# snuspl/parallax

Hardware: NVIDIA H100
Metric: lm1b_words_per_sec (higher is better)
Workload: dtype bf16

## Files before the change

parallax_b200/ops/csrc/kernels/lstm_softmax.cu:

```cuda
#include "common.cuh"

template <typename T> __device__ __forceinline__ float to_f(T v);
template <> __device__ __forceinline__ float to_f<float>(float v) { return v; }
template <> __device__ __forceinline__ float to_f<__nv_bfloat16>(__nv_bfloat16 v) { return __bfloat162float(v); }
template <typename T> __device__ __forceinline__ T from_f(float v);
template <> __device__ __forceinline__ float from_f<float>(float v) { return v; }
template <> __device__ __forceinline__ __nv_bfloat16 from_f<__nv_bfloat16>(float v) { return __float2bfloat16_rn(v); }

__device__ __forceinline__ float sigmoidf_(float x) { return 1.f / (1.f + __expf(-x)); }
__device__ __forceinline__ float tanhf_(float x) {
  const float e = __expf(-2.f * fabsf(x));
  const float t = (1.f - e) / (1.f + e);
  return copysignf(t, x);
}

template <typename T>
__global__ void __launch_bounds__(256)
px_lstm_cell_fwd_kernel(const T* __restrict__ gates, const float* __restrict__ c_prev,
                        T* __restrict__ act, float* __restrict__ c_new, T* __restrict__ m,
                        int B, int S, float forget_bias) {
  const int total = B * S;
  for (int idx = blockIdx.x * blockDim.x + threadIdx.x; idx < total;
       idx += gridDim.x * blockDim.x) {
    const int b = idx / S, s = idx - b * S;
    const size_t g0 = (size_t)b * 4 * S + s;
    const float si = sigmoidf_(to_f(gates[g0]));
    const float tj = tanhf_(to_f(gates[g0 + S]));
    const float sf = sigmoidf_(to_f(gates[g0 + 2 * S]) + forget_bias);
    const float so = sigmoidf_(to_f(gates[g0 + 3 * S]));
    const float c = sf * c_prev[idx] + si * tj;
    c_new[idx] = c;
    m[idx] = from_f<T>(so * tanhf_(c));
    act[g0] = from_f<T>(si);
    act[g0 + S] = from_f<T>(tj);
    act[g0 + 2 * S] = from_f<T>(sf);
    act[g0 + 3 * S] = from_f<T>(so);
  }
}

template <typename T>
__global__ void __launch_bounds__(256)
px_lstm_cell_bwd_kernel(const T* __restrict__ dm, float* __restrict__ dc,
                        const T* __restrict__ act, const float* __restrict__ c_prev,
                        const float* __restrict__ c_new, T* __restrict__ dgates, int B, int S) {
  const int total = B * S;
  for (int idx = blockIdx.x * blockDim.x + threadIdx.x; idx < total;
       idx += gridDim.x * blockDim.x) {
    const int b = idx / S, s = idx - b * S;
    const size_t g0 = (size_t)b * 4 * S + s;
    const float si = to_f(act[g0]), tj = to_f(act[g0 + S]), sf = to_f(act[g0 + 2 * S]),
                so = to_f(act[g0 + 3 * S]);
    const float tc = tanhf_(c_new[idx]);
    const float dmv = to_f(dm[idx]);
    const float dcv = dc[idx] + dmv * so * (1.f - tc * tc);
    dgates[g0] = from_f<T>(dcv * tj * si * (1.f - si));
    dgates[g0 + S] = from_f<T>(dcv * si * (1.f - tj * tj));
    dgates[g0 + 2 * S] = from_f<T>(dcv * c_prev[idx] * sf * (1.f - sf));
    dgates[g0 + 3 * S] = from_f<T>(dmv * tc * so * (1.f - so));
    dc[idx] = dcv * sf;
  }
}

template <typename T, int ITEMS, bool DOT>
__global__ void __launch_bounds__(256)
px_sampled_softmax_kernel(T* __restrict__ logits, const float* __restrict__ true_dot,
                          const float* __restrict__ adj_true,
                          const float* __restrict__ adj_samp,
                          const long long* __restrict__ targets, const long long* __restrict__ sampled,
                          float* __restrict__ loss, float* __restrict__ dtrue, int N, int S,
                          const T* __restrict__ h, const T* __restrict__ w_true, int P) {
  const int row = blockIdx.x;
  if (row >= N) return;
  __shared__ float s_red[8];
  __shared__ float s_bcast;
  T* x = logits + (size_t)row * S;
  const long long tgt = targets[row];
  float tl;
  if (DOT) {
    __shared__ float s_dot[8];
    const T* hr = h + (size_t)row * P;
    const T* wr = w_true + (size_t)row * P;
    float part = 0.f;
    for (int k = threadIdx.x; k < P; k += 256) part += to_f(hr[k]) * to_f(wr[k]);
    part = warp_sum(part);
    if ((threadIdx.x & 31) == 0) s_dot[threadIdx.x >> 5] = part;
    __syncthreads();
    float t = 0.f;
#pragma unroll
    for (int k = 0; k < 8; ++k) t += s_dot[k];
    tl = t + adj_true[row];
  } else {
    tl = true_dot[row] + adj_true[row];
  }
  float v[ITEMS];
  float mx = tl;
#pragma unroll
  for (int k = 0; k < ITEMS; ++k) {
    const int j = k * 256 + threadIdx.x;
    float a = -INFINITY;
    if (j < S) {
      a = to_f(x[j]) + adj_samp[j];
      if (sampled[j] == tgt) a = -INFINITY;
    }
    v[k] = a;
    mx = fmaxf(mx, a);
  }
  for (int o = 16; o > 0; o >>= 1) mx = fmaxf(mx, __shfl_xor_sync(0xffffffffu, mx, o));
  if ((threadIdx.x & 31) == 0) s_red[threadIdx.x >> 5] = mx;
  __syncthreads();
  if (threadIdx.x < 32) {
    float t = threadIdx.x < 8 ? s_red[threadIdx.x] : -INFINITY;
    for (int o = 4; o > 0; o >>= 1) t = fmaxf(t, __shfl_xor_sync(0xffffffffu, t, o));
    if (threadIdx.x == 0) s_bcast = t;
  }
  __syncthreads();
  mx = s_bcast;
  float sum = 0.f;
#pragma unroll
  for (int k = 0; k < ITEMS; ++k) { v[k] = __expf(v[k] - mx); sum += v[k]; }
  sum = warp_sum(sum);
  __syncthreads();
  if ((threadIdx.x & 31) == 0) s_red[threadIdx.x >> 5] = sum;
  __syncthreads();
  if (threadIdx.x < 32) {
    float t = threadIdx.x < 8 ? s_red[threadIdx.x] : 0.f;
    t = warp_sum(t);
    if (threadIdx.x == 0) s_bcast = t + __expf(tl - mx);
  }
  __syncthreads();
  const float denom = s_bcast;
  const float inv = 1.f / denom;
#pragma unroll
  for (int k = 0; k < ITEMS; ++k) {
    const int j = k * 256 + threadIdx.x;
    if (j < S) x[j] = from_f<T>(v[k] * inv);
  }
  if (threadIdx.x == 0) {
    loss[row] = (mx + __logf(denom)) - tl;
    dtrue[row] = __expf(tl - mx) * inv - 1.f;
  }
}

template <typename T> struct PxVec16;
template <> struct PxVec16<float> {
  static constexpr int N = 4;
  float v[4];
  __device__ __forceinline__ void load(const float* p) {
    const float4 t = *reinterpret_cast<const float4*>(p);
    v[0] = t.x; v[1] = t.y; v[2] = t.z; v[3] = t.w;
  }
  __device__ __forceinline__ void store(float* p) const {
    *reinterpret_cast<float4*>(p) = make_float4(v[0], v[1], v[2], v[3]);
  }
};
template <> struct PxVec16<__nv_bfloat16> {
  static constexpr int N = 8;
  float v[8];
  __device__ __forceinline__ void load(const __nv_bfloat16* p) {
    const uint4 t = *reinterpret_cast<const uint4*>(p);
    const unsigned w[4] = {t.x, t.y, t.z, t.w};
#pragma unroll
    for (int i = 0; i < 4; ++i) {
      v[2 * i] = __uint_as_float(w[i] << 16);
      v[2 * i + 1] = __uint_as_float(w[i] & 0xffff0000u);
    }
  }
  __device__ __forceinline__ void store(__nv_bfloat16* p) const {
    unsigned w[4];
#pragma unroll
    for (int i = 0; i < 4; ++i) {
      const __nv_bfloat162 b = __floats2bfloat162_rn(v[2 * i], v[2 * i + 1]);
      w[i] = *reinterpret_cast<const unsigned*>(&b);
    }
    *reinterpret_cast<uint4*>(p) = make_uint4(w[0], w[1], w[2], w[3]);
  }
};

template <typename T>
__global__ void __launch_bounds__(256)
px_ssm_bwd_kernel(T* __restrict__ G, const T* __restrict__ inputs, const T* __restrict__ w_true,
                  const float* __restrict__ g, int g_stride, const float* __restrict__ row_w,
                  const float* __restrict__ dtrue, float inv_n, T* __restrict__ gi,
                  T* __restrict__ d_w_true, void* __restrict__ d_b_true, int db_bf16,
                  T* __restrict__ grow_out, int N, int P) {
  constexpr int V = PxVec16<T>::N;
  const int per_row = P / V;
  const long long total = (long long)N * per_row;
  for (long long idx = (long long)blockIdx.x * blockDim.x + threadIdx.x; idx < total;
       idx += (long long)gridDim.x * blockDim.x) {
    const int row = (int)(idx / per_row);
    const int col = (int)(idx - (long long)row * per_row);
    float grow = g[(size_t)row * g_stride] * inv_n;
    if (row_w != nullptr) grow *= row_w[row];
    const float gt = grow * dtrue[row];
    const size_t off = (size_t)row * P + (size_t)col * V;
    PxVec16<T> a, x, w, o;
    a.load(G + off);
    x.load(inputs + off);
    w.load(w_true + off);
#pragma unroll
    for (int i = 0; i < V; ++i) o.v[i] = a.v[i] * grow + gt * w.v[i];
    o.store(G + off);
#pragma unroll
    for (int i = 0; i < V; ++i) o.v[i] = x.v[i] * grow;
    o.store(gi + off);
#pragma unroll
    for (int i = 0; i < V; ++i) o.v[i] = x.v[i] * gt;
    o.store(d_w_true + off);
    if (col == 0) {
      if (db_bf16) reinterpret_cast<__nv_bfloat16*>(d_b_true)[row] = __float2bfloat16_rn(gt);
      else reinterpret_cast<float*>(d_b_true)[row] = gt;
      grow_out[row] = from_f<T>(grow);
    }
  }
}

extern "C" {

int px_lstm_cell_fwd(const void* gates, const float* c_prev, void* act, float* c_new, void* m,
                     int B, int S, float forget_bias, int dtype, cudaStream_t stream) {
  int blocks = (B * S + 255) / 256;
  if (blocks > PX_NUM_SMS * 8) blocks = PX_NUM_SMS * 8;
  if (dtype == 0)
    px_lstm_cell_fwd_kernel<float><<<blocks, 256, 0, stream>>>(
        (const float*)gates, c_prev, (float*)act, c_new, (float*)m, B, S, forget_bias);
  else
    px_lstm_cell_fwd_kernel<__nv_bfloat16><<<blocks, 256, 0, stream>>>(
        (const __nv_bfloat16*)gates, c_prev, (__nv_bfloat16*)act, c_new, (__nv_bfloat16*)m, B, S,
        forget_bias);
  return (int)cudaGetLastError();
}

int px_lstm_cell_bwd(const void* dm, float* dc, const void* act, const float* c_prev,
                     const float* c_new, void* dgates, int B, int S, int dtype, cudaStream_t stream) {
  int blocks = (B * S + 255) / 256;
  if (blocks > PX_NUM_SMS * 8) blocks = PX_NUM_SMS * 8;
  if (dtype == 0)
    px_lstm_cell_bwd_kernel<float><<<blocks, 256, 0, stream>>>(
        (const float*)dm, dc, (const float*)act, c_prev, c_new, (float*)dgates, B, S);
  else
    px_lstm_cell_bwd_kernel<__nv_bfloat16><<<blocks, 256, 0, stream>>>(
        (const __nv_bfloat16*)dm, dc, (const __nv_bfloat16*)act, c_prev, c_new,
        (__nv_bfloat16*)dgates, B, S);
  return (int)cudaGetLastError();
}

int px_sampled_softmax(void* logits, const float* true_dot, const float* adj_true,
                       const float* adj_samp, const long long* targets, const long long* sampled,
                       float* loss, float* dtrue, int N, int S, int dtype, cudaStream_t stream) {
  if (S > 256 * 64) return -2;
#define SS(T, I)                                                                          \
  px_sampled_softmax_kernel<T, I, false><<<N, 256, 0, stream>>>(                          \
      (T*)logits, true_dot, adj_true, adj_samp, targets, sampled, loss, dtrue, N, S,      \
      (const T*)nullptr, (const T*)nullptr, 0)
#define SSD(T)                                                      \
  if (S <= 256 * 4) SS(T, 4); else if (S <= 256 * 8) SS(T, 8);      \
  else if (S <= 256 * 16) SS(T, 16); else if (S <= 256 * 32) SS(T, 32); else SS(T, 64)
  if (dtype == 0) { SSD(float); } else { SSD(__nv_bfloat16); }
#undef SSD
#undef SS
  return (int)cudaGetLastError();
}

int px_sampled_softmax_dot(void* logits, const void* h, const void* w_true, int P,
                           const float* adj_true, const float* adj_samp,
                           const long long* targets, const long long* sampled, float* loss,
                           float* dtrue, int N, int S, int dtype, cudaStream_t stream) {
  if (S > 256 * 64) return -2;
#define SS(T, I)                                                                          \
  px_sampled_softmax_kernel<T, I, true><<<N, 256, 0, stream>>>(                           \
      (T*)logits, nullptr, adj_true, adj_samp, targets, sampled, loss, dtrue, N, S,       \
      (const T*)h, (const T*)w_true, P)
#define SSD(T)                                                      \
  if (S <= 256 * 4) SS(T, 4); else if (S <= 256 * 8) SS(T, 8);      \
  else if (S <= 256 * 16) SS(T, 16); else if (S <= 256 * 32) SS(T, 32); else SS(T, 64)
  if (dtype == 0) { SSD(float); } else { SSD(__nv_bfloat16); }
#undef SSD
#undef SS
  return (int)cudaGetLastError();
}

int px_ssm_bwd(void* G, const void* inputs, const void* w_true, const float* g, int g_stride,
               const float* row_w, const float* dtrue, float inv_n, void* gi, void* d_w_true,
               void* d_b_true, int db_bf16, void* grow_out, int N, int P, int dtype,
               cudaStream_t stream) {
  const int vec = dtype == 0 ? 4 : 8;
  if (P % vec) return -2;
  const long long total = (long long)N * (P / vec);
  int blocks = (int)((total + 255) / 256);
  if (blocks > PX_NUM_SMS * 8) blocks = PX_NUM_SMS * 8;
  if (blocks < 1) blocks = 1;
  if (dtype == 0)
    px_ssm_bwd_kernel<float><<<blocks, 256, 0, stream>>>(
        (float*)G, (const float*)inputs, (const float*)w_true, g, g_stride, row_w, dtrue, inv_n,
        (float*)gi, (float*)d_w_true, d_b_true, db_bf16, (float*)grow_out, N, P);
  else
    px_ssm_bwd_kernel<__nv_bfloat16><<<blocks, 256, 0, stream>>>(
        (__nv_bfloat16*)G, (const __nv_bfloat16*)inputs, (const __nv_bfloat16*)w_true, g,
        g_stride, row_w, dtrue, inv_n, (__nv_bfloat16*)gi, (__nv_bfloat16*)d_w_true, d_b_true,
        db_bf16, (__nv_bfloat16*)grow_out, N, P);
  return (int)cudaGetLastError();
}

}
```

parallax_b200/ops/fused.py:

```python
import ctypes

import torch

from . import lib as _lib, check as _check, register_signatures

_vp, _i, _f = ctypes.c_void_p, ctypes.c_int, ctypes.c_float
register_signatures({
    "px_lstm_cell_fwd": (_i, [_vp, _vp, _vp, _vp, _vp, _i, _i, _f, _i, _vp]),
    "px_lstm_cell_bwd": (_i, [_vp, _vp, _vp, _vp, _vp, _vp, _i, _i, _i, _vp]),
    "px_sampled_softmax": (_i, [_vp, _vp, _vp, _vp, _vp, _vp, _vp, _vp, _i, _i, _i, _vp]),
    "px_sampled_softmax_dot": (_i, [_vp, _vp, _vp, _i, _vp, _vp, _vp, _vp, _vp, _vp, _i, _i, _i,
                                    _vp]),
    "px_ssm_bwd": (_i, [_vp, _vp, _vp, _vp, _i, _vp, _vp, _f, _vp, _vp, _vp, _i, _vp, _i, _i, _i,
                        _vp]),
})
_DT = {torch.float32: 0, torch.bfloat16: 1}


def _p(t):
    return _vp(t.data_ptr())


def _stream():
    return _vp(torch.cuda.current_stream().cuda_stream)


def _count(n=1):
    from ..parallel import nvops
    nvops.launches["n"] += n


def _acc(t):
    return t if t.dtype == torch.float64 else t.float()


def lstm_layer_reference(x, Wx, Wh, bias, W_P, c0, h0, forget_bias=1.0):
    T, Bsz, E = x.shape
    S = W_P.shape[0]
    xw = torch.addmm(bias, x.reshape(T * Bsz, E), Wx).view(T, Bsz, 4 * S)
    c, h, outs = _acc(c0), h0, []
    for t in range(T):
        gates = _acc(torch.addmm(xw[t], h, Wh))
        i, j, f, o = gates.split(S, dim=1)
        c = torch.sigmoid(f + forget_bias) * c + torch.sigmoid(i) * torch.tanh(j)
        m = (torch.sigmoid(o) * torch.tanh(c)).to(x.dtype)
        h = m @ W_P
        outs.append(h)
    return torch.stack(outs), c, h


class _LSTMLayerFn(torch.autograd.Function):

    @staticmethod
    def forward(ctx, x, W, Wh, bias, W_P, c0, h0, forget_bias):
        L = _lib()
        T, Bsz, E = x.shape
        S, P = W_P.shape
        dt = x.dtype
        dev = x.device
        x = x.contiguous()
        stacked = Wh is None
        ctx.stacked = stacked
        ctx.param_refs = (W, bias, W_P)
        if stacked:
            Wx, Wh = W.detach()[:E], W.detach()[E:]
        else:
            Wx = W
        if any(ctx.needs_input_grad):
            from . import sinks
            cur = torch.cuda.current_stream(dev)
            ws = sinks.side_stream(dev)
            ws.wait_stream(cur)
            with torch.cuda.stream(ws):
                ctx.WPT = W_P.detach().t().contiguous()
                ctx.WPT_ev = torch.cuda.Event()
                ctx.WPT_ev.record(ws)
            ctx.WPT.record_stream(cur)
        xw = torch.addmm(bias, x.view(T * Bsz, E), Wx).view(T, Bsz, 4 * S)
        act = torch.empty(T, Bsz, 4 * S, dtype=dt, device=dev)
        c_all = torch.empty(T + 1, Bsz, S, dtype=torch.float32, device=dev)
        m_all = torch.empty(T, Bsz, S, dtype=dt, device=dev)
        h_all = torch.empty(T + 1, Bsz, P, dtype=dt, device=dev)
        c_all[0].copy_(c0)
        h_all[0].copy_(h0)
        st = _stream()
        for t in range(T):
            gpre = xw[t].addmm_(h_all[t], Wh)
            _check(L.px_lstm_cell_fwd(_p(gpre), _p(c_all[t]), _p(act[t]),
                                      _p(c_all[t + 1]), _p(m_all[t]), Bsz, S,
                                      float(forget_bias), _DT[dt], st), "lstm_cell_fwd")
            torch.mm(m_all[t], W_P, out=h_all[t + 1])
        _count(T)
        ctx.save_for_backward(x, Wx, Wh, W_P, act, c_all, m_all, h_all)
        ctx.dims = (T, Bsz, E, S, P)
        return h_all[1:], c_all[T].clone(), h_all[T].clone()

    @staticmethod
    def backward(ctx, dH, dcT, dhT):
        from . import sinks
        L = _lib()
        x, Wx, Wh, W_P, act, c_all, m_all, h_all = ctx.saved_tensors
        T, Bsz, E, S, P = ctx.dims
        stacked = ctx.stacked
        W_ref, bias_ref, WP_ref = ctx.param_refs
        dt, dev = x.dtype, x.device
        dH = dH.contiguous()
        dgates = torch.empty(T, Bsz, 4 * S, dtype=dt, device=dev)
        dh_tot = torch.empty(T, Bsz, P, dtype=dt, device=dev)
        dc = torch.zeros(Bsz, S, dtype=torch.float32, device=dev) if dcT is None \
            else dcT.float().clone()
        dh_rec = None if dhT is None else dhT.to(dt)
        dm = torch.empty(Bsz, S, dtype=dt, device=dev)
        cur = torch.cuda.current_stream(dev)
        cur.wait_event(ctx.WPT_ev)
        WPT = ctx.WPT
        from . import gemm as _gemm
        use_tc = (dt == torch.bfloat16 and Bsz % 128 == 0 and P % 64 == 0 and
                  (4 * S) % 1024 == 0 and Wh.is_contiguous())
        WhT = None if use_tc else Wh.t().contiguous()
        st = _stream()

        def sink_of(ref, shape):
            s_ = sinks.get(ref)
            if s_ is not None and s_.dtype == dt and tuple(s_.shape) == tuple(shape):
                return s_, True
            return torch.empty(shape, dtype=dt, device=dev), False
        if stacked:
            dW, w_sunk = sink_of(W_ref, (E + P, 4 * S))
            dWx_o, dWh_o = dW[:E], dW[E:]
        else:
            dWx_o, w_sunk = sink_of(W_ref, (E, 4 * S))
            dWh_o = torch.empty(P, 4 * S, dtype=dt, device=dev)
        dbias_o, b_sunk = sink_of(bias_ref, (4 * S,))
        dWP_o, p_sunk = sink_of(WP_ref, (S, P))
        ws = sinks.side_stream(dev)
        ws2 = sinks.side_stream(dev, 1)
        if dh_rec is None:
            dh_tot[T - 1].copy_(dH[T - 1])
        else:
            torch.add(dH[T - 1], dh_rec, out=dh_tot[T - 1])
        for t in range(T - 1, -1, -1):
            torch.mm(dh_tot[t], WPT, out=dm)
            _check(L.px_lstm_cell_bwd(_p(dm), _p(dc), _p(act[t]), _p(c_all[t]),
                                      _p(c_all[t + 1]), _p(dgates[t]), Bsz, S, _DT[dt], st),
                   "lstm_cell_bwd")
            if t > 0:
                if use_tc:
                    _gemm.gemm_tn(dgates[t], Wh, addend=dH[t - 1], splits=8, bn=64,
                                  out=dh_tot[t - 1])
                else:
                    torch.addmm(dH[t - 1], dgates[t], WhT, out=dh_tot[t - 1])
            else:
                dh_rec = _gemm.gemm_tn(dgates[0], Wh, splits=8, bn=64) if use_tc \
                    else torch.mm(dgates[0], WhT)
        _count(T)
        dg2 = dgates.view(T * Bsz, 4 * S)
        ws2.wait_stream(cur)
        with torch.cuda.stream(ws2):
            torch.sum(dg2, 0, out=dbias_o)
        ev_b = torch.cuda.Event()
        ev_b.record(ws2)
        dgates.record_stream(ws2)
        dbias_o.record_stream(ws2)
        dx = (dg2 @ Wx.t()).view(T, Bsz, E)
        ws.wait_stream(cur)
        with torch.cuda.stream(ws):
            torch.mm(h_all[:T].reshape(-1, P).t(), dg2, out=dWh_o)
            torch.mm(x.reshape(-1, E).t(), dg2, out=dWx_o)
            torch.mm(m_all.reshape(-1, S).t(), dh_tot.view(-1, P), out=dWP_o)
        ev = torch.cuda.Event()
        ev.record(ws)
        for t_ in (dgates, dh_tot, x, h_all, m_all, dWh_o, dWx_o, dbias_o, dWP_o):
            t_.record_stream(ws)
        outs, plain = [], False
        for ref, o, sunk, e_ in ((W_ref, dW if stacked else dWx_o, w_sunk, ev),
                                 (bias_ref, dbias_o, b_sunk, ev_b), (WP_ref, dWP_o, p_sunk, ev)):
            if sunk:
                sinks.deliver(ref, e_)
                outs.append(None)
            else:
                outs.append(o)
                plain = True
        if plain or not stacked:
            cur.wait_event(ev)
            cur.wait_event(ev_b)
        dW_out, dbias, dW_P = outs
        return dx, dW_out, None if stacked else dWh_o, dbias, dW_P, dc, dh_rec, None


def lstm_layer(x, Wx, Wh, bias, W_P, c0, h0, forget_bias=1.0):
    if x.is_cuda and x.dtype in _DT:
        return _LSTMLayerFn.apply(x, Wx, Wh, bias, W_P, c0, h0, forget_bias)
    return lstm_layer_reference(x, Wx, Wh, bias, W_P, c0, h0, forget_bias)


def lstm_layer_stacked(x, W, bias, W_P, c0, h0, forget_bias=1.0):
    E = x.shape[-1]
    if x.is_cuda and x.dtype in _DT:
        return _LSTMLayerFn.apply(x, W, None, bias, W_P, c0, h0, forget_bias)
    return lstm_layer_reference(x, W[:E], W[E:], bias, W_P, c0, h0, forget_bias)


def sampled_softmax_reference(inputs, true_w, samp_w, true_b, samp_b, logq_true,
                              logq_samp, targets, sampled):
    true_logits = _acc((inputs * true_w).sum(-1)) + _acc(true_b) - logq_true
    samp_logits = _acc(inputs @ samp_w.t()) + (_acc(samp_b) - logq_samp)
    hits = targets.unsqueeze(1) == sampled.unsqueeze(0)
    samp_logits = samp_logits.masked_fill(hits, float("-inf"))
    lse = torch.logsumexp(torch.cat([true_logits.unsqueeze(1), samp_logits], 1), 1)
    return lse - true_logits


class _SampledSoftmaxFn(torch.autograd.Function):
    @staticmethod
    def forward(ctx, inputs, true_w, samp_w, true_b, samp_b, logq_true, logq_samp,
                targets, sampled):
        L = _lib()
        N, S = inputs.shape[0], samp_w.shape[0]
        dt = inputs.dtype
        logits = inputs @ samp_w.t()
        true_dot = (inputs.float() * true_w.float()).sum(-1)
        adj_t = (true_b.float() - logq_true).contiguous()
        adj_s = (samp_b.float() - logq_samp).contiguous()
        loss = torch.empty(N, dtype=torch.float32, device=inputs.device)
        dtrue = torch.empty(N, dtype=torch.float32, device=inputs.device)
        tg = targets.to(torch.int64).contiguous()
        sm = sampled.to(torch.int64).contiguous()
        _check(L.px_sampled_softmax(_p(logits), _p(true_dot), _p(adj_t), _p(adj_s), _p(tg),
                                    _p(sm), _p(loss), _p(dtrue), N, S, _DT[dt], _stream()),
               "sampled_softmax")
        _count(1)
        ctx.save_for_backward(inputs, true_w, samp_w, logits, dtrue)
        return loss

    @staticmethod
    def backward(ctx, g):
        inputs, true_w, samp_w, probs, dtrue = ctx.saved_tensors
        dt = inputs.dtype
        g = g.float()
        gt = (g * dtrue).unsqueeze(1)
        d_inputs = ((probs @ samp_w).float() * g.unsqueeze(1) +
                    gt * true_w.float()).to(dt)
        gi = (inputs.float() * g.unsqueeze(1)).to(dt)
        d_samp_w = probs.t() @ gi
        d_true_w = (gt * inputs.float()).to(dt)
        d_samp_b = (probs.float().t() @ g) if probs.dtype == torch.float32 else \
            torch.mm(probs.t(), g.to(dt).unsqueeze(1), out_dtype=torch.float32).squeeze(1)
        d_true_b = gt.squeeze(1)
        return d_inputs, d_true_w, d_samp_w, d_true_b, d_samp_b, None, None, None, None


def sampled_softmax_loss(inputs, true_w, samp_w, true_b, samp_b, logq_true, logq_samp,
                         targets, sampled):
    if inputs.is_cuda and inputs.dtype in _DT and samp_w.shape[0] <= 256 * 64:
        return _SampledSoftmaxFn.apply(inputs, true_w.to(inputs.dtype),
                                       samp_w.to(inputs.dtype), true_b, samp_b,
                                       logq_true, logq_samp, targets, sampled)
    return sampled_softmax_reference(inputs, true_w, samp_w, true_b, samp_b, logq_true,
                                     logq_samp, targets, sampled)


def _head_forward(inputs, w_all, adj, targets, sampled):
    N, S = inputs.shape[0], w_all.shape[0] - inputs.shape[0]
    P = inputs.shape[1]
    logits = inputs @ w_all[N:].t()
    if inputs.is_cuda:
        loss = torch.empty(N, dtype=torch.float32, device=inputs.device)
        dtrue = torch.empty(N, dtype=torch.float32, device=inputs.device)
        _check(_lib().px_sampled_softmax_dot(
            _p(logits), _p(inputs), _p(w_all), P, _p(adj), _vp(adj.data_ptr() + 4 * N),
            _p(targets), _p(sampled), _p(loss), _p(dtrue), N, S, _DT[inputs.dtype], _stream()),
            "sampled_softmax_dot")
        _count(1)
        return logits, loss, dtrue
    tl = (inputs.float() * w_all[:N].float()).sum(-1) + adj[:N]
    a = logits.float() + adj[N:]
    a = a.masked_fill(targets.unsqueeze(1) == sampled.unsqueeze(0), float("-inf"))
    mx = torch.maximum(a.max(1).values, tl)
    e, et = torch.exp(a - mx.unsqueeze(1)), torch.exp(tl - mx)
    denom = e.sum(1) + et
    return (e / denom.unsqueeze(1)).to(inputs.dtype), mx + torch.log(denom) - tl, et / denom - 1.0


def _head_backward(G, inputs, w_all, g, row_w, dtrue, gi, d_w_all, db, grow):
    N, P = inputs.shape
    if inputs.is_cuda:
        _check(_lib().px_ssm_bwd(
            _p(G), _p(inputs), _p(w_all), _p(g), 0 if g.numel() == 1 else 1,
            _p(row_w) if row_w is not None else None, _p(dtrue), 1.0 / N, _p(gi), _p(d_w_all),
            _p(db), 1 if db.dtype == torch.bfloat16 else 0, _p(grow), N, P, _DT[inputs.dtype],
            _stream()), "ssm_bwd")
        _count(1)
        return
    gr = g.reshape(-1).float() * (1.0 / N)
    gr = gr.expand(N) if gr.numel() == 1 else gr
    if row_w is not None:
        gr = gr * row_w
    gt = gr * dtrue
    x, wt = inputs.float(), w_all[:N].float()
    G.copy_(G.float() * gr.unsqueeze(1) + gt.unsqueeze(1) * wt)
    gi.copy_(x * gr.unsqueeze(1))
    d_w_all[:N].copy_(x * gt.unsqueeze(1))
    db[:N].copy_(gt)
    grow.copy_(gr)


class _SampledSoftmaxHeadFn(torch.autograd.Function):

    @staticmethod
    def forward(ctx, inputs, w_all, b_all, adj, targets, sampled, row_w):
        probs, loss, dtrue = _head_forward(inputs, w_all, adj, targets, sampled)
        ctx.save_for_backward(inputs, w_all, probs, dtrue, row_w)
        ctx.b_meta = (tuple(b_all.shape), b_all.dtype)
        if row_w is not None:
            loss = loss * row_w
        return loss.mean()

    @staticmethod
    def backward(ctx, g):
        inputs, w_all, probs, dtrue, row_w = ctx.saved_tensors
        N, P = inputs.shape
        S = w_all.shape[0] - N
        dt, dev = inputs.dtype, inputs.device
        b_shape, b_dt = ctx.b_meta
        g = g.float().contiguous()
        G = probs @ w_all[N:]
        d_w_all = torch.empty(N + S, P, dtype=dt, device=dev)
        db = torch.empty(N + S, dtype=b_dt if b_dt in _DT else torch.float32, device=dev)
        gi = torch.empty(N, P, dtype=dt, device=dev)
        grow = torch.empty(N, dtype=dt, device=dev)
        _head_backward(G, inputs, w_all, g, row_w, dtrue, gi, d_w_all, db, grow)
        torch.mm(probs.t(), gi, out=d_w_all[N:])
        if db.dtype == dt:
            torch.mm(probs.t(), grow.view(N, 1), out=db[N:].view(S, 1))
        elif dt == torch.bfloat16 and db.dtype == torch.float32:
            db[N:].copy_(torch.mm(probs.t(), grow.view(N, 1), out_dtype=torch.float32).view(S))
        else:
            db[N:].copy_((probs.t() @ grow.view(N, 1)).view(S))
        db = db.view(b_shape)
        if db.dtype != b_dt:
            db = db.to(b_dt)
        return G, d_w_all, db, None, None, None, None


def sampled_softmax_head(inputs, w_all, b_all, logq, targets, sampled, row_w=None, adj=None):
    N, P = inputs.shape
    S = w_all.shape[0] - N
    dt = inputs.dtype
    vec = 4 if dt == torch.float32 else 8
    fused = (inputs.is_cuda and dt in _DT and w_all.dtype == dt and
             0 < S <= 256 * 64 and P % vec == 0 and b_all.numel() == N + S)
    if fused:
        inputs = inputs.contiguous()
        w_all = w_all.contiguous()
        fused = inputs.data_ptr() % 16 == 0 and w_all.data_ptr() % 16 == 0
    if not fused:
        b = b_all.reshape(-1)
        loss = sampled_softmax_loss(inputs, w_all[:N], w_all[N:], b[:N], b[N:], logq[:N],
                                    logq[N:], targets, sampled)
        if row_w is not None:
            loss = loss * row_w.to(loss.dtype)
        return loss.mean()
    if adj is None:
        adj = b_all.detach().reshape(-1).float() - logq
    adj = adj.float().contiguous()
    tg = targets.to(torch.int64).contiguous()
    sm = sampled.to(torch.int64).contiguous()
    rw = None if row_w is None else row_w.detach().float().contiguous()
    return _SampledSoftmaxHeadFn.apply(inputs, w_all, b_all, adj, tg, sm, rw)
```

Measured before the change: 1.864 million.

## Fuse LSTM backward recurrence into a persistent cooperative kernel with grid barriers

Replaces the per-timestep loop of three launches (dm GEMM, cell backward, dh GEMM) with one cooperative persistent kernel. Each block keeps slices of W_P and Wh resident in shared memory, computes the dm projection with mma.sync, applies the cell backward math, then does a split-K dh GEMM with a workspace reduction, using software grid barriers between phases. This removes per-step launch overhead and repeated weight reloads, in exchange for grid-wide barrier latency and shape restrictions; unsupported shapes fall back to the old loop. It also factors the cell math into a shared header.

Result: faster. 1.916 million (median of 6 runs) (+2.8%).

```diff
diff --git a/parallax_b200/ops/csrc/kernels/lstm_cell.cuh b/parallax_b200/ops/csrc/kernels/lstm_cell.cuh
--- /dev/null
+++ b/parallax_b200/ops/csrc/kernels/lstm_cell.cuh
@@ -0,0 +1,34 @@
+#pragma once
+#include "common.cuh"
+
+__device__ __forceinline__ float sigmoidf_(float x) { return 1.f / (1.f + __expf(-x)); }
+__device__ __forceinline__ float tanhf_(float x) {
+  const float e = __expf(-2.f * fabsf(x));
+  const float t = (1.f - e) / (1.f + e);
+  return copysignf(t, x);
+}
+
+__device__ __forceinline__ void lstm_cell_fwd_math(float gi, float gj, float gf, float go,
+                                                   float c_prev, float forget_bias, float& si,
+                                                   float& tj, float& sf, float& so, float& c,
+                                                   float& m) {
+  si = sigmoidf_(gi);
+  tj = tanhf_(gj);
+  sf = sigmoidf_(gf + forget_bias);
+  so = sigmoidf_(go);
+  c = sf * c_prev + si * tj;
+  m = so * tanhf_(c);
+}
+
+__device__ __forceinline__ void lstm_cell_bwd_math(float si, float tj, float sf, float so,
+                                                   float c_prev, float c_new, float dmv,
+                                                   float dc_next, float (&dg)[4],
+                                                   float& dc_prev) {
+  const float tc = tanhf_(c_new);
+  const float dcv = dc_next + dmv * so * (1.f - tc * tc);
+  dg[0] = dcv * tj * si * (1.f - si);
+  dg[1] = dcv * si * (1.f - tj * tj);
+  dg[2] = dcv * c_prev * sf * (1.f - sf);
+  dg[3] = dmv * tc * so * (1.f - so);
+  dc_prev = dcv * sf;
+}
diff --git a/parallax_b200/ops/csrc/kernels/lstm_persistent.cu b/parallax_b200/ops/csrc/kernels/lstm_persistent.cu
--- /dev/null
+++ b/parallax_b200/ops/csrc/kernels/lstm_persistent.cu
@@ -0,0 +1,360 @@
+#include <map>
+#include <mutex>
+#include <set>
+#include <tuple>
+
+#include "lstm_cell.cuh"
+
+namespace lp {
+
+constexpr int WARPS = 8;
+constexpr int THREADS = WARPS * 32;
+constexpr int CH = 64;
+constexpr int NST = 4;
+constexpr int STAGE_BYTES = 16 * CH * 2;
+constexpr int STAGING = WARPS * NST * STAGE_BYTES;
+constexpr int UNITS = 16;
+constexpr int KS_BWD = 16;
+constexpr size_t CTR_BYTES = 32 * 4;
+
+__device__ __forceinline__ uint32_t smem_u32(const void* p) {
+  return (uint32_t)__cvta_generic_to_shared(p);
+}
+__device__ __forceinline__ uint32_t swz(int r, int c, int row_chunks) {
+  return (uint32_t)((r * row_chunks + (c ^ (r & 7))) * 16);
+}
+__device__ __forceinline__ void cp_async16(uint32_t dst, const void* src) {
+  asm volatile("cp.async.cg.shared.global [%0], [%1], 16;" ::"r"(dst), "l"(src) : "memory");
+}
+__device__ __forceinline__ void cp_async_commit() {
+  asm volatile("cp.async.commit_group;" ::: "memory");
+}
+template <int N>
+__device__ __forceinline__ void cp_async_wait() {
+  asm volatile("cp.async.wait_group %0;" ::"n"(N) : "memory");
+}
+__device__ __forceinline__ void ldmatrix_x4(uint32_t addr, uint32_t (&r)[4]) {
+  asm volatile("ldmatrix.sync.aligned.m8n8.x4.shared.b16 {%0,%1,%2,%3}, [%4];"
+               : "=r"(r[0]), "=r"(r[1]), "=r"(r[2]), "=r"(r[3]) : "r"(addr));
+}
+__device__ __forceinline__ void mma_bf16(float (&d)[4], const uint32_t (&a)[4], uint32_t b0,
+                                         uint32_t b1) {
+  asm volatile(
+      "mma.sync.aligned.m16n8k16.row.col.f32.bf16.bf16.f32 "
+      "{%0,%1,%2,%3}, {%4,%5,%6,%7}, {%8,%9}, {%0,%1,%2,%3};"
+      : "+f"(d[0]), "+f"(d[1]), "+f"(d[2]), "+f"(d[3])
+      : "r"(a[0]), "r"(a[1]), "r"(a[2]), "r"(a[3]), "r"(b0), "r"(b1));
+}
+__device__ __forceinline__ float bf16r(float v) {
+  return __bfloat162float(__float2bfloat16_rn(v));
+}
+__device__ __forceinline__ float2 ld_bf16x2(const __nv_bfloat16* p) {
+  return __bfloat1622float2(*reinterpret_cast<const __nv_bfloat162*>(p));
+}
+__device__ __forceinline__ void st_bf16x2(__nv_bfloat16* p, float a, float b) {
+  *reinterpret_cast<__nv_bfloat162*>(p) = __floats2bfloat162_rn(a, b);
+}
+
+__device__ __forceinline__ void bar_sync(unsigned int* ctr, bool leader, unsigned int n) {
+  __syncthreads();
+  if (threadIdx.x == 0) {
+    const unsigned int add = leader ? 0x80000000u - (n - 1u) : 1u;
+    __threadfence();
+    const unsigned int old = atomicAdd(ctr, add);
+    unsigned int cur;
+    do {
+      asm volatile("ld.acquire.gpu.global.u32 %0, [%1];" : "=r"(cur) : "l"(ctr) : "memory");
+    } while (((old ^ cur) & 0x80000000u) == 0u);
+    __threadfence();
+  }
+  __syncthreads();
+}
+
+template <int NT>
+__device__ __forceinline__ void warp_gemm(float (&acc)[NT][4], const __nv_bfloat16* A, int lda,
+                                          int K, uint32_t ring, uint32_t bs, int b_chunks) {
+  const int lane = threadIdx.x & 31;
+#pragma unroll
+  for (int nt = 0; nt < NT; ++nt)
+#pragma unroll
+    for (int e = 0; e < 4; ++e) acc[nt][e] = 0.f;
+  const int nch = K / CH;
+  auto load = [&](int ch) {
+    const uint32_t st = ring + (ch % NST) * STAGE_BYTES;
+#pragma unroll
+    for (int i = lane; i < 16 * (CH / 8); i += 32) {
+      const int r = i / (CH / 8), c = i % (CH / 8);
+      cp_async16(st + swz(r, c, CH / 8), A + (size_t)r * lda + ch * CH + c * 8);
+    }
+  };
+#pragma unroll
+  for (int s = 0; s < NST - 1; ++s) {
+    if (s < nch) load(s);
+    cp_async_commit();
+  }
+  for (int ch = 0; ch < nch; ++ch) {
+    if (ch + NST - 1 < nch) load(ch + NST - 1);
+    cp_async_commit();
+    cp_async_wait<NST - 1>();
+    __syncwarp();
+    const uint32_t st = ring + (ch % NST) * STAGE_BYTES;
+#pragma unroll
+    for (int kk = 0; kk < CH / 16; ++kk) {
+      uint32_t a[4];
+      ldmatrix_x4(st + swz(lane & 15, kk * 2 + (lane >> 4), CH / 8), a);
+      const int kc = ch * (CH / 8) + kk * 2;
+      const int mi = lane >> 3;
+#pragma unroll
+      for (int nt = 0; nt < NT; nt += 2) {
+        uint32_t b[4];
+        ldmatrix_x4(bs + swz((nt + (mi >> 1)) * 8 + (lane & 7), kc + (mi & 1), b_chunks), b);
+        mma_bf16(acc[nt], a, b[0], b[1]);
+        mma_bf16(acc[nt + 1], a, b[2], b[3]);
+      }
+    }
+    __syncwarp();
+  }
+}
+
+__device__ __forceinline__ void load_rows(uint8_t* bs, const __nv_bfloat16* src, size_t ld,
+                                          int rows, int K) {
+  const int chunks = K / 8;
+  for (int i = threadIdx.x; i < rows * chunks; i += THREADS) {
+    const int r = i / chunks, c = i % chunks;
+    *reinterpret_cast<uint4*>(bs + swz(r, c, chunks)) =
+        *reinterpret_cast<const uint4*>(src + (size_t)r * ld + c * 8);
+  }
+}
+template <int KS>
+__device__ __forceinline__ void split_reduce(const float (&acc)[8][4], float* ws,
+                                             unsigned int* tile_ctr, int nb, int ks, int B,
+                                             int P, const __nv_bfloat16* addend,
+                                             __nv_bfloat16* out) {
+  const int warp = threadIdx.x >> 5, lane = threadIdx.x & 31;
+  if (warp * 16 < B) {
+#pragma unroll
+    for (int nt = 0; nt < 8; ++nt)
+#pragma unroll
+      for (int h = 0; h < 2; ++h) {
+        const int row = warp * 16 + (lane >> 2) + 8 * h;
+        const int col = nb * 64 + nt * 8 + 2 * (lane & 3);
+        *reinterpret_cast<float2*>(ws + ((size_t)ks * B + row) * P + col) =
+            make_float2(acc[nt][2 * h], acc[nt][2 * h + 1]);
+      }
+  }
+  bar_sync(tile_ctr, ks == 0, KS);
+  constexpr int ROWS = 128 / KS;
+  for (int v = threadIdx.x; v < ROWS * 16; v += THREADS) {
+    const int row = ks * ROWS + v / 16, col = nb * 64 + (v % 16) * 4;
+    if (row >= B) continue;
+    float4 s = make_float4(0.f, 0.f, 0.f, 0.f);
+#pragma unroll
+    for (int p = 0; p < KS; ++p) {
+      const float4 x = __ldcg(reinterpret_cast<const float4*>(ws + ((size_t)p * B + row) * P + col));
+      s.x += x.x; s.y += x.y; s.z += x.z; s.w += x.w;
+    }
+    const size_t off = (size_t)row * P + col;
+    if (addend) {
+      const float2 lo = ld_bf16x2(addend + off), hi = ld_bf16x2(addend + off + 2);
+      s.x += lo.x; s.y += lo.y; s.z += hi.x; s.w += hi.y;
+    }
+    st_bf16x2(out + off, s.x, s.y);
+    st_bf16x2(out + off + 2, s.z, s.w);
+  }
+}
+
+struct BwdArgs {
+  const __nv_bfloat16* dH;
+  const __nv_bfloat16* Wh;
+  const __nv_bfloat16* WP;
+  const __nv_bfloat16* act;
+  const float* c_all;
+  __nv_bfloat16* dgates;
+  __nv_bfloat16* dh_tot;
+  __nv_bfloat16* dh_rec;
+  float* dc;
+  float* ws;
+  unsigned int* ctr;
+  int T, B, S, P;
+};
+
+__global__ void __launch_bounds__(THREADS, 1) px_lstm_bwd_persistent_kernel(BwdArgs a) {
+  extern __shared__ __align__(128) uint8_t smem[];
+  const int j = blockIdx.x, G = gridDim.x;
+  const int warp = threadIdx.x >> 5, lane = threadIdx.x & 31;
+  const int B = a.B, S = a.S, P = a.P, S4 = 4 * S;
+  const int ntiles = P / 64, Kb = S4 / KS_BWD;
+  const bool proj = j < ntiles * KS_BWD;
+  const int nb = j % ntiles, ks = j / ntiles;
+  uint8_t* s_wp = smem;
+  uint8_t* s_wh = s_wp + UNITS * P * 2;
+  const uint32_t ring = smem_u32(s_wh + 64 * Kb * 2) + warp * NST * STAGE_BYTES;
+  load_rows(s_wp, a.WP + (size_t)UNITS * j * P, (size_t)P, UNITS, P);
+  if (proj) load_rows(s_wh, a.Wh + (size_t)nb * 64 * S4 + (size_t)ks * Kb, (size_t)S4, 64, Kb);
+  __syncthreads();
+
+  const bool rows_on = warp * 16 < B;
+  const int g = lane >> 2, q = lane & 3;
+  float dc[2][2][2];
+  if (rows_on) {
+#pragma unroll
+    for (int rr = 0; rr < 2; ++rr)
+#pragma unroll
+      for (int nt = 0; nt < 2; ++nt) {
+        const float2 v = *reinterpret_cast<const float2*>(
+            a.dc + (size_t)(warp * 16 + g + 8 * rr) * S + UNITS * j + 8 * nt + 2 * q);
+        dc[rr][nt][0] = v.x; dc[rr][nt][1] = v.y;
+      }
+  }
+  unsigned int* grid_ctr = a.ctr;
+  for (int t = a.T - 1; t >= 0; --t) {
+    if (rows_on) {
+      float acc[2][4];
+      warp_gemm<2>(acc, a.dh_tot + ((size_t)t * B + warp * 16) * P, P, P, ring, smem_u32(s_wp),
+                   P / 8);
+#pragma unroll
+      for (int rr = 0; rr < 2; ++rr) {
+        const int b = warp * 16 + g + 8 * rr;
+        const size_t grow = ((size_t)t * B + b) * S4;
+#pragma unroll
+        for (int nt = 0; nt < 2; ++nt) {
+          const int s = UNITS * j + 8 * nt + 2 * q;
+          float2 av[4];
+#pragma unroll
+          for (int gt = 0; gt < 4; ++gt) av[gt] = ld_bf16x2(a.act + grow + (size_t)gt * S + s);
+          const float2 cp = *reinterpret_cast<const float2*>(a.c_all + ((size_t)t * B + b) * S + s);
+          const float2 cn =
+              *reinterpret_cast<const float2*>(a.c_all + ((size_t)(t + 1) * B + b) * S + s);
+          float dg0[4], dg1[4];
+          lstm_cell_bwd_math(av[0].x, av[1].x, av[2].x, av[3].x, cp.x, cn.x,
+                             bf16r(acc[nt][2 * rr]), dc[rr][nt][0], dg0, dc[rr][nt][0]);
+          lstm_cell_bwd_math(av[0].y, av[1].y, av[2].y, av[3].y, cp.y, cn.y,
+                             bf16r(acc[nt][2 * rr + 1]), dc[rr][nt][1], dg1, dc[rr][nt][1]);
+#pragma unroll
+          for (int gt = 0; gt < 4; ++gt)
+            st_bf16x2(a.dgates + grow + (size_t)gt * S + s, dg0[gt], dg1[gt]);
+        }
+      }
+    }
+    bar_sync(grid_ctr, j == 0, G);
+    if (proj) {
+      float acc[8][4];
+      if (rows_on)
+        warp_gemm<8>(acc, a.dgates + ((size_t)t * B + warp * 16) * S4 + (size_t)ks * Kb, S4, Kb,
+                     ring, smem_u32(s_wh), Kb / 8);
+      split_reduce<KS_BWD>(acc, a.ws, a.ctr + 1 + nb, nb, ks, B, P,
+                           t > 0 ? a.dH + (size_t)(t - 1) * B * P : nullptr,
+                           t > 0 ? a.dh_tot + (size_t)(t - 1) * B * P : a.dh_rec);
+    }
+    if (t > 0) bar_sync(grid_ctr, j == 0, G);
+  }
+  if (rows_on) {
+#pragma unroll
+    for (int rr = 0; rr < 2; ++rr)
+#pragma unroll
+      for (int nt = 0; nt < 2; ++nt)
+        *reinterpret_cast<float2*>(a.dc + (size_t)(warp * 16 + g + 8 * rr) * S + UNITS * j +
+                                   8 * nt + 2 * q) = make_float2(dc[rr][nt][0], dc[rr][nt][1]);
+  }
+}
+
+size_t bwd_smem(int S, int P) { return (size_t)UNITS * P * 2 + (size_t)64 * (4 * S / KS_BWD) * 2 + STAGING; }
+
+int check_shape(int B, int S, int P) {
+  if (B != 64 && B != 128) return -1;
+  if (P <= 0 || P % 64 || S <= 0 || S % 256) return -1;
+  const int G = S / UNITS, ntiles = P / 64;
+  if (ntiles * KS_BWD > G) return -1;
+  if (1 + ntiles > (int)(CTR_BYTES / 4)) return -1;
+  static std::mutex mu;
+  static std::map<std::tuple<int, int, int>, int> cache;
+  static std::set<int> attr_set;
+  std::lock_guard<std::mutex> lock(mu);
+  int dev = 0;
+  cudaGetDevice(&dev);
+  const auto key = std::make_tuple(dev, S, P);
+  auto it = cache.find(key);
+  if (it != cache.end()) return it->second;
+  int sms = 0, optin = 0;
+  cudaDeviceGetAttribute(&sms, cudaDevAttrMultiProcessorCount, dev);
+  cudaDeviceGetAttribute(&optin, cudaDevAttrMaxSharedMemoryPerBlockOptin, dev);
+  const void* fn = (const void*)px_lstm_bwd_persistent_kernel;
+  const size_t sm = bwd_smem(S, P);
+  if (sm > (size_t)optin) return cache[key] = -2;
+  cudaError_t e = cudaSuccess;
+  if (!attr_set.count(dev)) {
+    e = cudaFuncSetAttribute(fn, cudaFuncAttributeMaxDynamicSharedMemorySize, optin);
+    if (e == cudaSuccess) attr_set.insert(dev);
+  }
+  int per_sm = 0;
+  if (e == cudaSuccess) e = cudaOccupancyMaxActiveBlocksPerMultiprocessor(&per_sm, fn, THREADS, sm);
+  if (e != cudaSuccess) {
+    cudaGetLastError();
+    return cache[key] = -2;
+  }
+  return cache[key] = per_sm * sms < G ? -2 : 0;
+}
+
+unsigned int* barrier_ctrs(cudaStream_t stream) {
+  cudaStreamCaptureStatus status = cudaStreamCaptureStatusNone;
+  unsigned long long capture = 0;
+  if (cudaStreamGetCaptureInfo(stream, &status, &capture) != cudaSuccess) return nullptr;
+  if (status != cudaStreamCaptureStatusActive) capture = 0;
+  static std::mutex mu;
+  static std::map<std::tuple<int, cudaStream_t, unsigned long long>, unsigned int*> sets;
+  static std::map<int, cudaStream_t> zero_streams;
+  std::lock_guard<std::mutex> lock(mu);
+  int dev = 0;
+  cudaGetDevice(&dev);
+  const auto key = std::make_tuple(dev, stream, capture);
+  auto it = sets.find(key);
+  if (it != sets.end()) return it->second;
+  cudaStreamCaptureMode mode = cudaStreamCaptureModeRelaxed;
+  cudaThreadExchangeStreamCaptureMode(&mode);
+  void* p = nullptr;
+  cudaError_t e = cudaMalloc(&p, CTR_BYTES);
+  if (e == cudaSuccess && !zero_streams.count(dev)) {
+    cudaStream_t zs;
+    e = cudaStreamCreateWithFlags(&zs, cudaStreamNonBlocking);
+    if (e == cudaSuccess) zero_streams[dev] = zs;
+  }
+  if (e == cudaSuccess) e = cudaMemsetAsync(p, 0, CTR_BYTES, zero_streams[dev]);
+  if (e == cudaSuccess) e = cudaStreamSynchronize(zero_streams[dev]);
+  cudaThreadExchangeStreamCaptureMode(&mode);
+  if (e != cudaSuccess) {
+    cudaGetLastError();
+    if (p) cudaFree(p);
+    return nullptr;
+  }
+  return sets[key] = (unsigned int*)p;
+}
+
+}
+
+extern "C" {
+
+int px_lstm_persistent_supported(int B, int S, int P) { return lp::check_shape(B, S, P) == 0; }
+
+void* px_lstm_barrier_ctrs(cudaStream_t stream) { return lp::barrier_ctrs(stream); }
+
+int px_lstm_bwd_persistent(const void* dH, const void* Wh, const void* WP, const void* act,
+                           const float* c_all, void* dgates, void* dh_tot, void* dh_rec,
+                           float* dc, float* ws, int T, int B, int S, int P, cudaStream_t stream) {
+  const int rc = lp::check_shape(B, S, P);
+  if (rc) return rc;
+  unsigned int* ctr = lp::barrier_ctrs(stream);
+  if (!ctr) return -5;
+  lp::BwdArgs a;
+  a.dH = (const __nv_bfloat16*)dH; a.Wh = (const __nv_bfloat16*)Wh;
+  a.WP = (const __nv_bfloat16*)WP; a.act = (const __nv_bfloat16*)act; a.c_all = c_all;
+  a.dgates = (__nv_bfloat16*)dgates; a.dh_tot = (__nv_bfloat16*)dh_tot;
+  a.dh_rec = (__nv_bfloat16*)dh_rec; a.dc = dc; a.ws = ws; a.ctr = ctr;
+  a.T = T; a.B = B; a.S = S; a.P = P;
+  void* args[] = {&a};
+  const cudaError_t e = cudaLaunchCooperativeKernel((const void*)lp::px_lstm_bwd_persistent_kernel,
+                                                    dim3(S / lp::UNITS), dim3(lp::THREADS), args,
+                                                    lp::bwd_smem(S, P), stream);
+  return e == cudaSuccess ? (int)cudaGetLastError() : (int)e;
+}
+
+}
diff --git a/parallax_b200/ops/csrc/kernels/lstm_softmax.cu b/parallax_b200/ops/csrc/kernels/lstm_softmax.cu
--- a/parallax_b200/ops/csrc/kernels/lstm_softmax.cu
+++ b/parallax_b200/ops/csrc/kernels/lstm_softmax.cu
@@ -1,4 +1,4 @@
-#include "common.cuh"
+#include "lstm_cell.cuh"
 
 template <typename T> __device__ __forceinline__ float to_f(T v);
 template <> __device__ __forceinline__ float to_f<float>(float v) { return v; }
@@ -6,13 +6,6 @@
 template <typename T> __device__ __forceinline__ T from_f(float v);
 template <> __device__ __forceinline__ float from_f<float>(float v) { return v; }
 template <> __device__ __forceinline__ __nv_bfloat16 from_f<__nv_bfloat16>(float v) { return __float2bfloat16_rn(v); }
-
-__device__ __forceinline__ float sigmoidf_(float x) { return 1.f / (1.f + __expf(-x)); }
-__device__ __forceinline__ float tanhf_(float x) {
-  const float e = __expf(-2.f * fabsf(x));
-  const float t = (1.f - e) / (1.f + e);
-  return copysignf(t, x);
-}
 
 template <typename T>
 __global__ void __launch_bounds__(256)
@@ -24,13 +17,11 @@
        idx += gridDim.x * blockDim.x) {
     const int b = idx / S, s = idx - b * S;
     const size_t g0 = (size_t)b * 4 * S + s;
-    const float si = sigmoidf_(to_f(gates[g0]));
-    const float tj = tanhf_(to_f(gates[g0 + S]));
-    const float sf = sigmoidf_(to_f(gates[g0 + 2 * S]) + forget_bias);
-    const float so = sigmoidf_(to_f(gates[g0 + 3 * S]));
-    const float c = sf * c_prev[idx] + si * tj;
+    float si, tj, sf, so, c, mv;
+    lstm_cell_fwd_math(to_f(gates[g0]), to_f(gates[g0 + S]), to_f(gates[g0 + 2 * S]),
+                       to_f(gates[g0 + 3 * S]), c_prev[idx], forget_bias, si, tj, sf, so, c, mv);
     c_new[idx] = c;
-    m[idx] = from_f<T>(so * tanhf_(c));
+    m[idx] = from_f<T>(mv);
     act[g0] = from_f<T>(si);
     act[g0 + S] = from_f<T>(tj);
     act[g0 + 2 * S] = from_f<T>(sf);
@@ -50,14 +41,11 @@
     const size_t g0 = (size_t)b * 4 * S + s;
     const float si = to_f(act[g0]), tj = to_f(act[g0 + S]), sf = to_f(act[g0 + 2 * S]),
                 so = to_f(act[g0 + 3 * S]);
-    const float tc = tanhf_(c_new[idx]);
-    const float dmv = to_f(dm[idx]);
-    const float dcv = dc[idx] + dmv * so * (1.f - tc * tc);
-    dgates[g0] = from_f<T>(dcv * tj * si * (1.f - si));
-    dgates[g0 + S] = from_f<T>(dcv * si * (1.f - tj * tj));
-    dgates[g0 + 2 * S] = from_f<T>(dcv * c_prev[idx] * sf * (1.f - sf));
-    dgates[g0 + 3 * S] = from_f<T>(dmv * tc * so * (1.f - so));
-    dc[idx] = dcv * sf;
+    float dg[4], dcp;
+    lstm_cell_bwd_math(si, tj, sf, so, c_prev[idx], c_new[idx], to_f(dm[idx]), dc[idx], dg, dcp);
+#pragma unroll
+    for (int g = 0; g < 4; ++g) dgates[g0 + g * S] = from_f<T>(dg[g]);
+    dc[idx] = dcp;
   }
 }
 
diff --git a/parallax_b200/ops/fused.py b/parallax_b200/ops/fused.py
--- a/parallax_b200/ops/fused.py
+++ b/parallax_b200/ops/fused.py
@@ -13,6 +13,10 @@
                                     _vp]),
     "px_ssm_bwd": (_i, [_vp, _vp, _vp, _vp, _i, _vp, _vp, _f, _vp, _vp, _vp, _i, _vp, _i, _i, _i,
                         _vp]),
+    "px_lstm_persistent_supported": (_i, [_i, _i, _i]),
+    "px_lstm_barrier_ctrs": (_vp, [_vp]),
+    "px_lstm_bwd_persistent": (_i, [_vp, _vp, _vp, _vp, _vp, _vp, _vp, _vp, _vp, _vp, _i, _i, _i,
+                                    _i, _vp]),
 })
 _DT = {torch.float32: 0, torch.bfloat16: 1}
 
@@ -49,6 +53,58 @@
     return torch.stack(outs), c, h
 
 
+_PERSISTENT_KS_BWD = 16
+
+
+def _persistent_ok(x, Wh, W_P):
+    T, Bsz, _ = x.shape
+    S, P = W_P.shape
+    return (x.is_cuda and T >= 1 and x.dtype == torch.bfloat16 and Wh.dtype == torch.bfloat16
+            and W_P.dtype == torch.bfloat16 and
+            bool(_lib().px_lstm_persistent_supported(Bsz, S, P)))
+
+
+def _recurrence_bwd_loop(dH, Wh, WPT, act, c_all, dgates, dh_tot, dc):
+    L = _lib()
+    T, Bsz, P = dH.shape
+    S = c_all.shape[2]
+    dt, dev = dH.dtype, dH.device
+    dm = torch.empty(Bsz, S, dtype=dt, device=dev)
+    from . import gemm as _gemm
+    use_tc = (dt == torch.bfloat16 and Bsz % 128 == 0 and P % 64 == 0 and
+              (4 * S) % 1024 == 0 and Wh.is_contiguous())
+    WhT = None if use_tc else Wh.t().contiguous()
+    st = _stream()
+    for t in range(T - 1, -1, -1):
+        torch.mm(dh_tot[t], WPT, out=dm)
+        _check(L.px_lstm_cell_bwd(_p(dm), _p(dc), _p(act[t]), _p(c_all[t]),
+                                  _p(c_all[t + 1]), _p(dgates[t]), Bsz, S, _DT[dt], st),
+               "lstm_cell_bwd")
+        if t > 0:
+            if use_tc:
+                _gemm.gemm_tn(dgates[t], Wh, addend=dH[t - 1], splits=8, bn=64,
+                              out=dh_tot[t - 1])
+            else:
+                torch.addmm(dH[t - 1], dgates[t], WhT, out=dh_tot[t - 1])
+        else:
+            dh_rec = _gemm.gemm_tn(dgates[0], Wh, splits=8, bn=64) if use_tc \
+                else torch.mm(dgates[0], WhT)
+    _count(T)
+    return dh_rec
+
+
+def _recurrence_bwd_persistent(dH, Wh, W_P, act, c_all, dgates, dh_tot, dc):
+    T, Bsz, P = dH.shape
+    S = W_P.shape[0]
+    dh_rec = torch.empty(Bsz, P, dtype=dH.dtype, device=dH.device)
+    ws = torch.empty(_PERSISTENT_KS_BWD, Bsz, P, dtype=torch.float32, device=dH.device)
+    _check(_lib().px_lstm_bwd_persistent(
+        _p(dH), _p(Wh), _p(W_P), _p(act), _p(c_all), _p(dgates), _p(dh_tot), _p(dh_rec), _p(dc),
+        _p(ws), T, Bsz, S, P, _stream()), "lstm_bwd_persistent")
+    _count(1)
+    return dh_rec
+
+
 class _LSTMLayerFn(torch.autograd.Function):
 
     @staticmethod
@@ -66,7 +122,9 @@
             Wx, Wh = W.detach()[:E], W.detach()[E:]
         else:
             Wx = W
-        if any(ctx.needs_input_grad):
+        Wh, W_P = Wh.contiguous(), W_P.contiguous()
+        ctx.persistent = persistent = _persistent_ok(x, Wh, W_P)
+        if any(ctx.needs_input_grad) and not persistent:
             from . import sinks
             cur = torch.cuda.current_stream(dev)
             ws = sinks.side_stream(dev)
@@ -98,7 +156,6 @@
     @staticmethod
     def backward(ctx, dH, dcT, dhT):
         from . import sinks
-        L = _lib()
         x, Wx, Wh, W_P, act, c_all, m_all, h_all = ctx.saved_tensors
         T, Bsz, E, S, P = ctx.dims
         stacked = ctx.stacked
@@ -110,15 +167,7 @@
         dc = torch.zeros(Bsz, S, dtype=torch.float32, device=dev) if dcT is None \
             else dcT.float().clone()
         dh_rec = None if dhT is None else dhT.to(dt)
-        dm = torch.empty(Bsz, S, dtype=dt, device=dev)
         cur = torch.cuda.current_stream(dev)
-        cur.wait_event(ctx.WPT_ev)
-        WPT = ctx.WPT
-        from . import gemm as _gemm
-        use_tc = (dt == torch.bfloat16 and Bsz % 128 == 0 and P % 64 == 0 and
-                  (4 * S) % 1024 == 0 and Wh.is_contiguous())
-        WhT = None if use_tc else Wh.t().contiguous()
-        st = _stream()
 
         def sink_of(ref, shape):
             s_ = sinks.get(ref)
@@ -139,21 +188,11 @@
             dh_tot[T - 1].copy_(dH[T - 1])
         else:
             torch.add(dH[T - 1], dh_rec, out=dh_tot[T - 1])
-        for t in range(T - 1, -1, -1):
-            torch.mm(dh_tot[t], WPT, out=dm)
-            _check(L.px_lstm_cell_bwd(_p(dm), _p(dc), _p(act[t]), _p(c_all[t]),
-                                      _p(c_all[t + 1]), _p(dgates[t]), Bsz, S, _DT[dt], st),
-                   "lstm_cell_bwd")
-            if t > 0:
-                if use_tc:
-                    _gemm.gemm_tn(dgates[t], Wh, addend=dH[t - 1], splits=8, bn=64,
-                                  out=dh_tot[t - 1])
-                else:
-                    torch.addmm(dH[t - 1], dgates[t], WhT, out=dh_tot[t - 1])
-            else:
-                dh_rec = _gemm.gemm_tn(dgates[0], Wh, splits=8, bn=64) if use_tc \
-                    else torch.mm(dgates[0], WhT)
-        _count(T)
+        if ctx.persistent:
+            dh_rec = _recurrence_bwd_persistent(dH, Wh, W_P, act, c_all, dgates, dh_tot, dc)
+        else:
+            cur.wait_event(ctx.WPT_ev)
+            dh_rec = _recurrence_bwd_loop(dH, Wh, ctx.WPT, act, c_all, dgates, dh_tot, dc)
         dg2 = dgates.view(T * Bsz, 4 * S)
         ws2.wait_stream(cur)
         with torch.cuda.stream(ws2):
```
